# Toytiny/CMFlow

Measured on AMD Instinct MI355X. Metric: frame-pairs/sec CMFlow fwd+bwd, higher is better.
Workload: dtype f32; 1 GPU; cmflow fwd+bwd training (7 cross-modal losses + Adam, train-mode BN) step, N=256, B=64 per GPU (global 64), ball-query r=2/4/8/16 K=4/8/16/32, kNN K=8; synthetic clouds, seeded random-init weights; parallelism=dp1

## Files before the change

cmflow_amd/_lib.py:

```python
import ctypes
import os
import subprocess

import torch

_HERE = os.path.dirname(os.path.abspath(__file__))
SO_PATH = os.environ.get("CMF_LIB") or os.path.join(_HERE, "libcmflow_hip.so")

_vp, _ci, _cf, _ll = ctypes.c_void_p, ctypes.c_int, ctypes.c_float, ctypes.c_longlong

SIGNATURES = {
    "cmf_ball_query": [_ci, _ci, _ci, _cf, _ci, _vp, _vp, _vp, _vp],
    "cmf_ball_query_multi": [_ci, _ci, _ci, _ci, _vp, _vp, _ci, _vp, _vp, _vp, _ci, _vp],
    "cmf_setconv_queries": [_ci, _vp, _vp],
    "cmf_ball_query_multi_counted": [_ci, _ci, _ci, _ci, _vp, _vp, _ci, _vp, _vp, _vp, _vp, _vp, _vp],
    "cmf_setconv_queries_counted": [_ci, _vp, _vp, _vp],
    "cmf_knn_counted": [_ci, _ci, _ci, _ci, _vp, _vp, _vp, _vp, _vp, _vp],
    "cmf_global_max_cat_counted": [_ci, _ci, _ci, _vp, _ll, _vp, _ll, _vp, _vp, _vp],
    "cmf_ego_refine_counted": [_ci, _ci, _cf, _cf, _vp, _vp, _vp, _vp, _vp, _vp, _vp, _vp, _vp, _vp, _vp, _vp],
    "cmf_eval_metrics_counted": [_ci, _ci, _vp, _vp, _vp, _vp, _vp, _vp, _vp, _vp, _cf, _cf, _cf, _vp, _vp, _vp],
    "cmf_ego_refine_grad_counted": [_ci, _ci, _cf, _vp, _vp, _vp, _vp, _vp, _vp, _vp, _vp, _vp, _vp, _vp, _vp, _vp],
    "cmf_global_max_cat_grad_counted": [_ci, _ci, _ci, _vp, _ll, _vp, _vp, _ll, _vp, _vp],
    "cmf_radar_loss_counted_workspace": [_ci, _ci, _ci, _ci],
    "cmf_radar_loss_counted_workspace_tiled": [_ci, _ci, _ci, _ci],
# ... 51 lines not shown
    "cmf_three_interpolate_grad": [_ci, _ci, _ci, _ci, _vp, _vp, _vp, _vp, _vp],
    "cmf_bn_finalize": [_ci, _ci, ctypes.c_double, _vp, _vp, _vp, _cf, _cf, _vp, _vp, _vp, _vp, _vp, _vp, _vp, _vp],
    "cmf_colsum_finalize": [_ci, _ci, _vp, _vp, _vp, _vp, _vp],
    "cmf_group_affine": [_ci, _ci, _ci, _ci, _ci, _vp, _ci, _vp, _ci, _vp, _vp, _vp, _ci, _vp, _ci, _vp, _vp, _vp, _vp, _vp],
    "cmf_adam_step": [_ci, _vp, _vp, _ll, _vp, _vp, _vp, ctypes.c_double, ctypes.c_double, ctypes.c_double, ctypes.c_double, ctypes.c_double, _ll, _vp],
    "cmf_grad_norm_parts": [_ll],
    "cmf_grad_sumsq": [_ll, _vp, _vp, _vp],
    "cmf_grad_norm": [_ll, _vp, _vp, _vp, _vp],
    "cmf_adam_step_guarded": [_ci, _vp, _vp, _ll, _vp, _vp, _vp, ctypes.c_double, ctypes.c_double, ctypes.c_double, ctypes.c_double, ctypes.c_double, _ll,
                              ctypes.c_double, _ci, _vp, _vp, _vp],
    "cmf_adam_step_ema": [_ci, _vp, _vp, _ll, _vp, _vp, _vp, ctypes.c_double, ctypes.c_double, ctypes.c_double, ctypes.c_double, ctypes.c_double, _ll,
                          _vp, ctypes.c_double, _vp],
    "cmf_adam_step_guarded_ema": [_ci, _vp, _vp, _ll, _vp, _vp, _vp, ctypes.c_double, ctypes.c_double, ctypes.c_double, ctypes.c_double, ctypes.c_double,
                                  _ll, ctypes.c_double, _ci, _vp, _vp, _vp, ctypes.c_double, _vp],
    "cmf_param_exchange": [_ci, _vp, _vp, _ll, _vp, _vp],
    "cmf_group_prep": [_ci, _ci, _ci, _ci, _ci, _vp, _vp, _vp, _ci, _vp, _vp, _vp, _vp, _vp],
    "cmf_gemm_gather_affine": [_ci, _ci, _ci, _vp, _ll, _vp, _vp, _vp, _vp, _vp, _vp, _ll, _vp, _ll, _vp, _vp],
    "cmf_gemm_dx_gather": [_ci, _ci, _ci, _vp, _ll, _vp, _ll, _vp, _ll, _vp, _ll, _vp, _vp, _vp, _vp, _vp, _vp, _vp, _vp, _vp],
    "cmf_group_perm": [_ci, _ci, _vp, _vp, _vp, _vp, _vp, _vp, _vp],
    "cmf_gemm_dx_gather_sum": [_ci, _ci, _ci, _vp, _ll, _vp, _ll, _vp, _ll, _vp, _vp, _vp, _vp, _vp, _vp, _vp, _vp, _vp, _vp, _vp],
    "cmf_group_rows_grad_bn_cf_pieces": [_ci, _ci, _ci, _ci, _ci, _vp, _vp, _ll, _vp, _ll, _vp, _vp, _vp, _vp, _vp, _vp, _cf, _vp, _vp, _vp,
                                         _ci, _vp],
    "cmf_gemm_dw_gather_split": [_ci, _ci, _ll],
    "cmf_gemm_dw_gather_bn_bwd": [_ci, _ci, _ll, _vp, _ll, _vp, _ll, _vp, _vp, _vp, _vp, _vp, _ll, _vp, _ll, _vp, _vp, _vp, _vp, _vp, _vp, _ll,
                                  _ci, _vp, _ci, _vp],
    "cmf_gemm_dw_gather": [_ci, _ci, _ll, _vp, _ll, _vp, _ll, _vp, _vp, _vp, _vp, _vp, _vp, _ll, _ci, _vp, _ci, _vp],
    "cmf_colsum": [_ci, _ci, _vp, _vp, _ci, _vp, _vp, _vp],
    "cmf_setconv_dwx": [_ci, _cf, _ci, _vp, _vp, _vp, _vp, _vp, _vp, _ci, _ci, _vp],
    "cmf_group_rows_grad_bn": [_ci, _ci, _ci, _ci, _vp, _vp, _vp, _vp, _vp, _vp, _cf, _vp, _vp, _vp, _ci, _vp],
    "cmf_group_rows_grad_bn_cf": [_ci, _ci, _ci, _ci, _ci, _vp, _vp, _ll, _vp, _ll, _vp, _vp, _vp, _vp, _vp, _vp, _cf, _vp, _vp, _vp,
                                  _ci, _vp],
    "cmf_bn_relu_maxpool": [_ll, _ci, _ci, _vp, _vp, _vp, _vp, _ll, _vp, _vp],
    "cmf_maxpool_bwd": [_ll, _ci, _ci, _vp, _ll, _vp, _vp, _vp, _vp, _vp, _vp, _vp, _vp, _vp],
    "cmf_affine_relu": [_ll, _ci, _vp, _ll, _vp, _vp, _vp, _ll, _vp],
    "cmf_act_bwd_stats": [_ll, _ci, _vp, _ll, _vp, _ll, _vp, _vp, _vp, _vp, _vp, _vp, _vp],
    "cmf_bn_bwd_apply": [_ll, _ci, _vp, _vp, _ll, _vp, _vp, _vp, _vp, _vp],
    "cmf_maxpool_bwd_point": [_ll, _ci, _ci, _vp, _ll, _vp, _vp, _vp, _vp, _vp, _vp, _vp, _vp, _vp],
    "cmf_thin_bwd_layer_pooled": [_ll, _ci, _ci, _ci, _vp, _vp, _vp, _vp, _vp, _vp, _vp, _vp, _vp, _vp, _vp, _vp, _vp, _vp, _vp, _vp,
                                  _ci, _vp, _vp],
    "cmf_thin_bwd_wide_supported": [_ci, _ci],
    "cmf_thin_bwd_wide_slabs": [_ll, _ci, _vp],
    "cmf_thin_bwd_wide_layer": [_ll, _ci, _vp, _ll, _vp, _vp, _ci, _vp, _ll, _vp, _vp, _vp, _vp, _vp, _ll, _vp, _ll,
                                _vp, _vp, _vp, _vp, _vp, _ll, _vp, _vp, _ll, _ci, _vp, _vp],
    "cmf_thin_bwd_supported": [_ci, _ci],
    "cmf_thin_bwd_slabs": [_ll, _vp],
    "cmf_thin_bwd_layer": [_ll, _ci, _ci, _vp, _ll, _vp, _ll, _vp, _vp, _vp, _vp, _vp, _ll, _vp, _ll, _ci,
                           _vp, _vp, _vp, _vp, _vp, _vp, _ll, _vp, _vp, _ll, _ci, _vp, _vp],
    "cmf_weighted_ksum": [_ll, _ci, _ci, _ci, _ci, _vp, _vp, _vp, _vp, _vp],
    "cmf_weighted_ksum_grad_tiles": [_ci],
    "cmf_weighted_ksum_grad": [_ll, _ci, _ci, _ci, _ci, _ci, _vp, _vp, _vp, _vp, _vp, _vp, _vp, _vp],
    "cmf_weightnet_ksum_tiles": [_ci],
    "cmf_weightnet_ksum": [_ll, _ci, _ci, _ci, _ci, _vp, _vp, _vp, _vp, _vp, _vp, _vp],
    "cmf_weightnet_ksum_grad": [_ll, _ci, _ci, _ci, _ci, _ci, _vp, _ll, _vp, _vp, _vp, _vp, _vp, _vp, _vp, _vp, _vp],
    "cmf_global_max_cat": [_ci, _ci, _ci, _vp, _ll, _vp, _ll, _vp, _vp],
    "cmf_stack_first_conv": [_ci, _ci, _ci, _ci, _ci, _vp, _vp, _vp],
    "cmf_unstack_first_conv_grad": [_ci, _ci, _ci, _ci, _ci, _vp, _vp, _vp],
    "cmf_global_max_cat_grad": [_ci, _ci, _ci, _vp, _ll, _vp, _vp, _ll, _vp],
    "cmf_mem_stats": [],
    "cmf_radar_loss_workspace_nb": [_ci, _ci, _ci],
    "cmf_radar_loss_workspace_tiled": [_ci, _ci, _ci],
    "cmf_radar_loss": [_vp, _vp],
    "cmf_radar_loss_tiled": [_vp, _vp],
    "cmf_pseudo_labels": [_ci, _ci, _vp, _vp, _vp, _vp, _vp, _vp, _cf, _vp, _vp, _vp, _vp],
    "cmf_draw_batch": [_ci, _ci, _ci, _ci, _vp, _vp, _vp, _vp, _vp, _vp, _vp, ctypes.c_ulonglong, ctypes.c_ulonglong,
                       _vp, _vp, _vp, _vp, _vp, _vp, _vp, _vp, _vp, _vp, _vp, _vp, _vp, _vp],
    "cmf_draw_batch_at": [_ci, _ci, _ci, _ci, _ci, _vp, _vp, _vp, _vp, _vp, _vp, _vp, ctypes.c_ulonglong, ctypes.c_ulonglong,
                          _vp, _vp, _vp, _vp, _vp, _vp, _vp, _vp, _vp, _vp, _vp, _vp, _vp, _vp],
    "cmf_draw_frames": [_ci, _ci, _ci, _ci, _vp, _vp, _vp, _vp, _vp, _vp, _vp,
                        _vp, _vp, _vp, _vp, _vp, _vp, _vp, _vp, _vp, _vp, _vp, _vp, _vp, _vp],
    "cmf_augment_batch": [_ci, _ci, _ci, _ci, ctypes.c_ulonglong, ctypes.c_ulonglong, ctypes.c_double, _ci, _vp, _vp, _vp, _vp, _vp, _vp, _vp, _vp],
    "cmf_prepare_count": [_ci, _ci, _vp, _vp, _vp, _vp, _ci, _ci, _ci, ctypes.c_double, ctypes.c_double, _vp, _vp, _vp, _vp],
    "cmf_prepare_scans": [_ci, _ci, _ci, _vp, _vp, _vp, _vp, _ci, _ci, _ci, ctypes.c_double, ctypes.c_double, _vp, _vp, _vp, _vp],
    "cmf_prepare_pairs": [_ci, _ci, _vp, _vp, _vp, _vp, _vp, _vp, _vp, _vp, _vp, _vp, _ci, _vp, _ci, _ci, _vp, _vp, _vp],
    "cmf_pack_results": [_ci, _ci, _ci, _vp, _vp, _vp, _ll, _vp, _vp, _vp, _vp, _vp, _vp, _vp, _vp, _vp, _vp, _vp, _vp],
    "cmf_eval_metrics_frames": [_ci, _ci, _vp, _vp, _vp, _vp, _vp, _vp, _vp, _vp, _cf, _cf, _cf, _ci, _vp, _vp, _vp, _vp],
    "cmf_pose_chain": [_ci, _ci, _vp, _vp, _vp, _vp],
    "cmf_debug_spin": [_cf, _vp],
    "cmf_eval_metrics": [_ci, _ci, _vp, _vp, _vp, _vp, _vp, _vp, _vp, _cf, _cf, _cf, _vp, _vp, _vp],
}
RESTYPES = {"cmf_mem_stats": _ll, "cmf_radar_loss_counted_workspace": _ll, "cmf_radar_loss_counted_workspace_tiled": _ll,
            "cmf_radar_loss_workspace_nb": _ll, "cmf_radar_loss_workspace_tiled": _ll, "cmf_gemm_trace_read": _ll, "cmf_gemm_profile_records": _ll}


class GemmLaunchRecord(ctypes.Structure):
    _fields_ = [("M", _ci), ("N", _ci), ("K", _ci), ("layout", _ci), ("split_k", _ci), ("kind", _ci), ("bm", _ci), ("bn", _ci),
                ("ms", _cf)]


class SetConvDesc(ctypes.Structure):
    _fields_ = [("B", _ci), ("N", _ci), ("S", _ci), ("O1", _ci), ("C", _ci * 5), ("radius", _cf), ("training", _ci),
                ("eps", _cf * 6), ("momentum", _cf * 6),
                ("xyz", _vp), ("y", _vp), ("ldy", _ll), ("wx", _vp), ("ldwx", _ll), ("w", _vp * 5),
                ("gamma", _vp * 6), ("beta", _vp * 6), ("rmean", _vp * 6), ("rvar", _vp * 6), ("nbt", _vp * 6),
                ("saved", _vp), ("scratch", _vp), ("out", _vp), ("ldo", _ll),
                ("dout", _vp), ("lddout", _ll), ("dy", _vp), ("lddy", _ll), ("dwx", _vp), ("lddwx", _ll), ("acc_wx", _ci),
                ("dw", _vp * 5), ("acc_w", _ci * 5), ("dgamma", _vp * 6), ("dbeta", _vp * 6), ("acc_bn", _ci * 6),
                ("inference", _ci), ("idx_ready", _ci)]


class MlpDesc(ctypes.Structure):
    _fields_ = [("M", _ll), ("L", _ci), ("C", _ci * 5), ("training", _ci), ("eps", _cf * 4), ("momentum", _cf * 4),
                ("x", _vp), ("ldx", _ll), ("w", _vp * 4), ("gamma", _vp * 4), ("beta", _vp * 4),
                ("rmean", _vp * 4), ("rvar", _vp * 4), ("nbt", _vp * 4), ("saved", _vp), ("scratch", _vp),
                ("out", _vp), ("ldo", _ll), ("dout", _vp), ("lddout", _ll), ("dx", _vp), ("lddx", _ll),
                ("dw", _vp * 4), ("acc_w", _ci * 4), ("dgamma", _vp * 4), ("dbeta", _vp * 4), ("acc_bn", _ci * 4)]

# ... 131 lines not shown
```

cmflow_amd/csrc/wsum.hip:

```cpp
#include "cmf_common.h"
#include "../../include/cmflow_hip.h"

constexpr int WS_THREADS = 256;

template <int KU>
__global__ __launch_bounds__(WS_THREADS) void wsum_fwd_kernel(
    long long M, int K, int C, int n1, int n_src, const float *__restrict__ w, const float *__restrict__ x,
    const int *__restrict__ idx, float *__restrict__ out)
{
    const int cv = C / 4;
    const long long total = M * cv;
    for (long long t = (long long)blockIdx.x * WS_THREADS + threadIdx.x; t < total; t += (long long)gridDim.x * WS_THREADS) {
        const long long m = t / cv;
        const int c = (int)(t - m * cv) * 4;
        const float *wp = w + (m * K) * C + c;
        const long long src_base = idx ? (m / n1) * n_src : 0;
        float4 acc = make_float4(0.f, 0.f, 0.f, 0.f);
        for (int k0 = 0; k0 < K; k0 += KU) {
            float4 wv[KU], xv[KU];
#pragma unroll
            for (int u = 0; u < KU; ++u) {
                const int k = k0 + u;
                if (k < K) {
                    wv[u] = *(const float4 *)(wp + (long long)k * C);
// ... 232 lines not shown
            q2[i] = keep + __shfl_xor(send, 16, 64);
        }
        {
            const float keep = up3 ? q2[1] : q2[0], send = up3 ? q2[0] : q2[1];
            q1 = keep + __shfl_xor(send, 8, 64);
        }
        q1 += __shfl_xor(q1, 4, 64);
        q1 += __shfl_xor(q1, 2, 64);
        q1 += __shfl_xor(q1, 1, 64);
        if ((lane & 7) == 0) sred[it & 1][wave][(lane >> 5) * 4 + ((lane >> 4) & 1) * 2 + ((lane >> 3) & 1)] = q1;
        __syncthreads();
        if (tid < R * WN_J) {
            const int rr = tid / WN_J, j = tid % WN_J;
            if (row0 + rr < MK) {
                float s = sred[it & 1][rr * wpr][j];
                for (int w = 1; w < wpr; ++w) s += sred[it & 1][rr * wpr + w][j];
                if (leaky & 4) {
                    s = h[(long long)(row0 + rr) * WN_J + j] > 0.f ? s : 0.f;
                    dbh += s;
                }
                dh[(long long)(row0 + rr) * WN_J + j] = s;
            }
        }
    }
    float *prow = part + (long long)blockIdx.x * (C * (WN_J + 2) + WN_J);
    {
        __syncthreads();
        float *fl = (float *)fold;
        if (tid < R * WN_J) fl[tid] = dbh;
        __syncthreads();
        if (tid < WN_J) {
            float t = fl[tid];
            for (int rr = 1; rr < R; ++rr) t += fl[rr * WN_J + tid];
            prow[C * (WN_J + 2) + tid] = t;
        }
    }
#pragma unroll
    for (int q = 0; q < 10; ++q) {
        float4 v;
        if (q < 8) { const int i = q >> 1, j = (q & 1) * 4; v = make_float4(dW[i][j], dW[i][j + 1], dW[i][j + 2], dW[i][j + 3]); }
        else if (q == 8) v = make_float4(db[0], db[1], db[2], db[3]);
        else v = make_float4(cs[0], cs[1], cs[2], cs[3]);
        __syncthreads();
        fold[tid] = v;
        __syncthreads();
        if (r == 0) {
            for (int rr = 1; rr < R; ++rr) { const float4 o = fold[tid + rr * cv]; v.x += o.x; v.y += o.y; v.z += o.z; v.w += o.w; }
            if (q < 8) *(float4 *)(prow + (c + (q >> 1)) * WN_J + (q & 1) * 4) = v;
            else *(float4 *)(prow + C * WN_J + (q - 8) * C + c) = v;
        }
    }
}

extern "C" int cmf_weightnet_ksum_tiles(int C)
{
    return (C == 256 || C == 512 || C == 1024) ? WN_TILES : 0;
}

extern "C" int cmf_weightnet_ksum(long long M, int K, int C, int n1, int n_src, const float *h, const float *Wl, const float *bl,
                                  const float *x, const int *idx, float *out, void *stream)
{
    CMF_CHECK_ARG(M >= 0 && K > 0 && cmf_weightnet_ksum_tiles(C) > 0 && M * K < (1LL << 31));
    if (M == 0) return 0;
    CMF_CHECK_ARG(h && Wl && bl && x && out && (!idx || (n1 > 0 && n_src > 0)));
    CMF_CHECK_ARG((((uintptr_t)h | (uintptr_t)Wl | (uintptr_t)x | (uintptr_t)out) & 15) == 0);
    const int R = WS_THREADS / (C / 4);
    const long long want = (M + R - 1) / R;
    const int grid = (int)(want < 2048 ? want : 2048);
    hipLaunchKernelGGL(wn_ksum_fwd_kernel, dim3(grid), dim3(WS_THREADS), 0, (hipStream_t)stream, (int)M, K, C, n1, n_src, h, Wl, bl, x, idx, out);
    return cmf_launch_status();
}

extern "C" int cmf_weightnet_ksum_grad(long long M, int K, int C, int n1, int n_src, int leaky, const float *dcost, long long ldd, const float *h,
                                       const float *Wl, const float *bl, const float *x, const int *idx, float *dx, float *dh,
                                       float *part, void *stream)
{
    CMF_CHECK_ARG(M >= 0 && K > 0 && cmf_weightnet_ksum_tiles(C) > 0 && M * K < (1LL << 31));
    CMF_CHECK_ARG(dcost && h && Wl && bl && x && dx && dh && part && (!idx || (n1 > 0 && n_src > 0)) && ldd >= C && ldd % 4 == 0);
    CMF_CHECK_ARG((((uintptr_t)h | (uintptr_t)Wl | (uintptr_t)x | (uintptr_t)dcost | (uintptr_t)dx | (uintptr_t)dh | (uintptr_t)part) & 15) == 0);
    hipLaunchKernelGGL(wn_ksum_bwd_kernel, dim3(WN_TILES), dim3(WS_THREADS), 0, (hipStream_t)stream, (int)M, K, C, n1, n_src, leaky, dcost, ldd, h,
                       Wl, bl, x, idx, dx, dh, part);
    return cmf_launch_status();
}
```

cmflow_amd/fused_blocks.py:

```python
import ctypes
import os

import torch
from torch.autograd import Function

from . import _lib
from . import pointnet2_utils as pointutils
from .fused import Neighbors, gemm, group_rows

_f32, _i32 = torch.float32, torch.int32
L = _lib.lib


def _p(t):
    return None if t is None else t.data_ptr()


def _tiles(M):
    return (M + 127) // 128


class BNState:
    __slots__ = ("a", "c", "mean", "invstd", "training", "count")

# ... 1128 lines not shown
        n_src = nbr.n if nbr is not None else 0
        part, db = None, None
        want_db = ctx.x_bias is not None and len(ctx.needs_input_grad) > 5 and ctx.needs_input_grad[5] and need_x
        tiles = L().cmf_weighted_ksum_grad_tiles(C) if want_db else 0
        if tiles > 0:
            part = torch.empty(tiles, 1, C, dtype=_f32, device=weights.device)
        _lib.check(L().cmf_weighted_ksum_grad(B * N1, K, C, N1, n_src, int(leaky), _p(dcost), _p(weights), _p(x), idx,
                                              _p(dw), _p(dx), _p(part), _lib.stream_ptr()), "cmf_weighted_ksum_grad")
        if want_db:
            if part is not None:
                sink = grad_sink(ctx.x_bias)
                sums = colsum_n(part, C, sink, None)
                db = None if sink is not None else sums.view(-1)
            else:
                db = dx.view(-1, C).sum(0)
        if nbr is not None and need_x:
            off, inv = nbr.inverse()
            dp = torch.empty(B, nbr.n, C, dtype=_f32, device=weights.device)
            _lib.check(L().cmf_group_rows_grad(B, nbr.n, C, C, N1 * K, 0, _p(dx), _p(off), _p(inv), _p(dp), _lib.stream_ptr()),
                       "cmf_group_rows_grad")
            dx = dp
        return dw, dx, None, None, None, db


class WeightNetKSumFn(Function):

    @staticmethod
    def supported(C, J):
        return J == 8 and L().cmf_weightnet_ksum_tiles(int(C)) > 0

    @staticmethod
    def forward(ctx, h, wl, bl, x, nbr, leaky, x_bias=None, h_bias=None):
        B, N1, K, J = h.shape
        C = wl.shape[0]
        h, wl, bl, x = h.contiguous(), wl.contiguous(), bl.contiguous(), x.contiguous()
        out = torch.empty(B, N1, C, dtype=_f32, device=h.device)
        idx = _lib.dev_ptr(nbr.idx, torch.int32) if nbr is not None else None
        n_src = nbr.n if nbr is not None else 0
        _lib.check(L().cmf_weightnet_ksum(B * N1, K, C, N1, n_src, _p(h), _p(wl), _p(bl), _p(x), idx, _p(out), _lib.stream_ptr()),
                   "cmf_weightnet_ksum")
        ctx.saved = (h, wl, bl, x, nbr, int(bool(leaky)) | (4 if h_bias is not None else 0))
        ctx.params = (wl, bl, x_bias, h_bias)
        return out

    @staticmethod
    def backward(ctx, dcost):
        h, wl, bl, x, nbr, leaky = ctx.saved
        B, N1, K, J = h.shape
        C = wl.shape[0]
        dev = h.device
        if not (dcost.stride(2) == 1 and dcost.stride(0) == N1 * dcost.stride(1) and dcost.stride(1) % 4 == 0
                and dcost.data_ptr() % 16 == 0):
            dcost = dcost.contiguous()
        dx = torch.empty(B, N1, K, C, dtype=_f32, device=dev)
        dh = torch.empty_like(h)
        part = torch.empty(L().cmf_weightnet_ksum_tiles(C), C * (J + 2) + J, dtype=_f32, device=dev)
        idx = _lib.dev_ptr(nbr.idx, torch.int32) if nbr is not None else None
        n_src = nbr.n if nbr is not None else 0
        _lib.check(L().cmf_weightnet_ksum_grad(B * N1, K, C, N1, n_src, leaky, dcost.data_ptr(), dcost.stride(1), _p(h), _p(wl), _p(bl), _p(x), idx,
                                               _p(dx), _p(dh), _p(part), _lib.stream_ptr()), "cmf_weightnet_ksum_grad")
        sums = colsum_n(part)
        grads = [sums[:C * J].view(C, J), sums[C * J:C * J + C], sums[C * J + C:C * J + 2 * C] if ctx.params[2] is not None else None,
                 sums[C * (J + 2):] if ctx.params[3] is not None else None]
        sinks = [grad_sink(p) if p is not None else None for p in ctx.params]
        pairs = [(s.view(-1), g.reshape(-1)) for s, g in zip(sinks, grads) if s is not None and g is not None]
        if pairs:
            torch._foreach_add_([s for s, _ in pairs], [g for _, g in pairs])
        dwl, dbl, dxb, dhb = [None if (s is not None or g is None) else g for s, g in zip(sinks, grads)]
        if nbr is not None:
            off, inv = nbr.inverse()
            dp = torch.empty(B, nbr.n, C, dtype=_f32, device=dev)
            _lib.check(L().cmf_group_rows_grad(B, nbr.n, C, C, N1 * K, 0, _p(dx), _p(off), _p(inv), _p(dp), _lib.stream_ptr()),
                       "cmf_group_rows_grad")
            dx = dp
        return dh, dwl, dbl, dx, None, None, dxb, dhb


class GlobalMaxCatFn(Function):

    @staticmethod
    def forward(ctx, f):
        B, N, C = f.shape
        f = f.contiguous()
        out = torch.empty(B, N, 2 * C, dtype=_f32, device=f.device)
        arg = torch.empty(B, C, dtype=torch.int32, device=f.device)
        _lib.check(L().cmf_global_max_cat(B, N, C, _p(f), C, _p(out), 2 * C, _p(arg), _lib.stream_ptr()), "cmf_global_max_cat")
        ctx.arg = arg
        return out

    @staticmethod
    def backward(ctx, dout):
        B, C = ctx.arg.shape
        N = dout.shape[1]
        if not (dout.stride(2) == 1 and dout.stride(0) == N * dout.stride(1) and dout.stride(1) % 4 == 0 and dout.data_ptr() % 16 == 0):
            dout = dout.contiguous()
        df = torch.empty(B, N, C, dtype=_f32, device=dout.device)
        _lib.check(L().cmf_global_max_cat_grad(B, N, C, dout.data_ptr(), dout.stride(1), _p(ctx.arg), _p(df), C, _lib.stream_ptr()),
                   "cmf_global_max_cat_grad")
        return df


def global_max_cat(f):
    return GlobalMaxCatFn.apply(f)


class GlobalMaxCatCountedFn(Function):

    @staticmethod
    def forward(ctx, f, counts):
        B, N, C = f.shape
        f = f.contiguous()
        out = torch.empty(B, N, 2 * C, dtype=_f32, device=f.device)
        arg = torch.empty(B, C, dtype=torch.int32, device=f.device)
        _lib.check(L().cmf_global_max_cat_counted(B, N, C, _p(f), C, _p(out), 2 * C, _p(arg), _lib.dev_ptr(counts, torch.int32),
                                                  _lib.stream_ptr()), "cmf_global_max_cat_counted")
        ctx.arg, ctx.counts = arg, counts
        return out

    @staticmethod
    def backward(ctx, dout):
        B, C = ctx.arg.shape
        N = dout.shape[1]
# ... 20 lines not shown
```

include/cmflow_hip.h:

```cpp
#ifndef CMFLOW_HIP_H
#define CMFLOW_HIP_H

#ifdef __cplusplus
extern "C" {
#endif


int cmf_ball_query(int b, int n, int m, float radius, int nsample,
                   const float *new_xyz, const float *xyz, int *idx, void *stream);
int cmf_ball_query_multi(int b, int n, int m, int nq, const float *radii, const int *nsamples, int nclouds,
                         const float *const *new_xyz, const float *const *xyz, int *const *idx, int zero_empty, void *stream);

int cmf_group_points(int b, int c, int n, int npoints, int nsample,
                     const float *points, const int *idx, float *out, void *stream);

int cmf_group_points_grad(int b, int c, int n, int npoints, int nsample,
                          const float *grad_out, const int *idx, float *grad_points, void *stream);

int cmf_query_and_group(int b, int n, int m, float radius, int nsample, int c, int use_xyz,
                        const float *new_xyz, const float *xyz, const float *features, int *idx, float *out, void *stream);


int cmf_knn(int b, int n, int s, int nsample, const float *xyz, const float *new_xyz,
            int *idx, float *dist, void *stream);
// ... 207 lines not shown
                      void *stream);
int cmf_adam_step_guarded_ema(int n_tensors, const long long *offsets, float *const *params, long long total, const float *grad, float *m,
                              float *v, double lr, double beta1, double beta2, double eps, double weight_decay, long long step,
                              double max_grad_norm, int skip_nonfinite, const double *partials, double *record, float *ema,
                              double ema_decay, void *stream);
int cmf_param_exchange(int n_tensors, const long long *offsets, float *const *params, long long total, float *flat, void *stream);

int cmf_setconv_bn_offsets(const cmf_setconv_desc *d, long long *offsets6);

typedef struct cmf_mlp_desc {
    long long M; int L; int C[5]; int training;
    float eps[4], momentum[4];
    const float *x; long long ldx;
    const float *w[4];
    const float *gamma[4], *beta[4];
    float *rmean[4], *rvar[4]; long long *nbt[4];
    float *saved, *scratch;
    float *out; long long ldo;
    const float *dout; long long lddout;
    float *dx; long long lddx;
    float *dw[4]; int acc_w[4];
    float *dgamma[4], *dbeta[4]; int acc_bn[4];
} cmf_mlp_desc;
int cmf_mlp_sizes(const cmf_mlp_desc *d, long long *saved_floats, long long *scratch_fwd, long long *scratch_bwd);
int cmf_mlp_forward(const cmf_mlp_desc *d, void *stream);
int cmf_mlp_backward(const cmf_mlp_desc *d, void *stream);

typedef struct cmf_bn_update_entry {
    float *rmean, *rvar; long long *nbt;
    int C; float momentum, eps; double count;
    long long offset;
} cmf_bn_update_entry;
int cmf_bn_running_update(int n_entries, const cmf_bn_update_entry *table, int n_calls, const float *saved0,
                          const float *saved1, void *stream);

int cmf_setconv_forward_heads_multi(int n, const cmf_setconv_desc *descs, void *const *streams);
int cmf_setconv_forward_bodies_batched(int n, const cmf_setconv_desc *descs);
int cmf_setconv_backward_bodies_batched(int n, const cmf_setconv_desc *descs);
int cmf_setconv_tail_forward(int n, const cmf_setconv_desc *descs, void *stream);
int cmf_setconv_tail_backward(int n, const cmf_setconv_desc *descs, void *stream);
int cmf_setconv_backward_bodies_multi(int n, const cmf_setconv_desc *descs, void *const *streams);

int cmf_weighted_ksum(long long M, int K, int C, int n1, int n_src, const float *w, const float *x, const int *idx,
                      float *out, void *stream);
int cmf_weighted_ksum_grad_tiles(int C);
int cmf_weighted_ksum_grad(long long M, int K, int C, int n1, int n_src, int leaky, const float *dcost, const float *w,
                           const float *x, const int *idx, float *dw, float *dx, float *dx_colsum, void *stream);
int cmf_weightnet_ksum_tiles(int C);
int cmf_weightnet_ksum(long long M, int K, int C, int n1, int n_src, const float *h, const float *Wl, const float *bl,
                       const float *x, const int *idx, float *out, void *stream);
int cmf_weightnet_ksum_grad(long long M, int K, int C, int n1, int n_src, int leaky, const float *dcost, long long ldd, const float *h,
                            const float *Wl, const float *bl, const float *x, const int *idx, float *dx, float *dh,
                            float *part, void *stream);

int cmf_global_max_cat(int B, int N, int C, const float *f, long long ldf, float *out, long long ldo, int *arg, void *stream);
int cmf_global_max_cat_grad(int B, int N, int C, const float *dout, long long ldd, const int *arg, float *df, long long ldf,
                            void *stream);

int cmf_stack_first_conv(int n_w, int O1, int cin, int n_tail, int Kp, const float *const *w, float *wf, void *stream);
int cmf_unstack_first_conv_grad(int n_w, int O1, int cin, int n_tail, int Kp, const float *dwf, float *const *g, void *stream);

#define CMF_RADAR_LOSS_MAX_N 65536
typedef struct cmf_radar_loss_desc {
    int B, N;
    const float *pc1, *pc2, *pred_f, *gt_f;
    const float *vel1, *mseg_pre, *mseg_gt, *dyn_mask, *radar_u, *radar_v;
    const float *opt;
    const float *pre_trans, *gt_trans;
    const float *camera_inverse;
    const float *t_camera_radar;
    float w_self, w_em, w_ms, w_opt, w_dyn;
    float zeta, alpha; int num_nb; float lower_bound;
    int self_only;
    float *items;
    float *d_pred_f, *d_pre_trans, *d_mseg_pre;
    float *workspace;
    const float *t_camera_radar_batch;
} cmf_radar_loss_desc;
long long cmf_radar_loss_workspace_nb(int b, int n, int num_nb);
int cmf_radar_loss(const cmf_radar_loss_desc *d, void *stream);
int cmf_radar_loss_tiled(const cmf_radar_loss_desc *d, void *stream);
long long cmf_radar_loss_workspace_tiled(int b, int n, int num_nb);

int cmf_eval_metrics(int b, int n, const float *pc, const float *pred, const float *labels, const float *mask,
                     const float *pred_m, const float *gt_trans, const float *pred_trans,
                     float r_res, float theta_res, float phi_res, double *metrics, double *workspace, void *stream);

int cmf_pseudo_labels(int b, int n, const float *pc1, const float *gt_trans, const float *vel1, const float *interval,
                      const float *fg_mask, const float *flow_label, float vr_thres,
                      float *dyn_mask, float *mseg_gt, float *residual, void *stream);

int cmf_debug_spin(float microseconds, void *stream);

int cmf_ball_query_multi_counted(int b, int n, int m, int nq, const float *radii, const int *nsamples, int nclouds,
                                 const float *const *new_xyz, const float *const *xyz, int *const *idx,
                                 const int *const *n_ctr, const int *const *n_src, void *stream);
int cmf_setconv_queries_counted(int n, const cmf_setconv_desc *descs, const int *const *counts, void *stream);
int cmf_knn_counted(int b, int n, int s, int nsample, const float *xyz, const float *new_xyz, const int *n_src,
                    int *idx, float *dist, void *stream);
int cmf_global_max_cat_counted(int B, int N, int C, const float *f, long long ldf, float *out, long long ldo, int *arg,
                               const int *cnt, void *stream);
int cmf_ego_refine_counted(int b, int n, float eps, float thres, const float *pc1, const float *flow, const float *score,
                           const int *cnt, float *W, float *Bm, float *trans, double *aux, float *sf, unsigned char *mask,
                           float *stat, void *stream);
int cmf_eval_metrics_counted(int b, int n, const int *cnt, const float *pc, const float *pred, const float *labels, const float *mask,
                             const float *pred_m, const float *gt_trans, const float *pred_trans,
// ... 90 lines not shown
```

Before: 3444 frame-pairs/s.

## Fuse weightnet ksum backward with neighbor scatter via inverse index lists

Adds a wave-per-row weightnet ksum backward kernel for C=256/512 with register-resident weights and a depth-2 load prefetch. Adds a scatter variant that walks each source point's inverse neighbor list and accumulates dx straight into per-point gradients. This removes the B×N1×K×C intermediate dx tensor and the separate group_rows_grad pass. In exchange the code is more complex, depends on the inverse-list layout, and risks load imbalance across waves when neighbor lists vary in length.

Result: no change. 3464 frame-pairs/s, median of 6 (+0.6%).

```diff
diff --git a/cmflow_amd/_lib.py b/cmflow_amd/_lib.py
--- a/cmflow_amd/_lib.py
+++ b/cmflow_amd/_lib.py
@@ -127,6 +127,8 @@
     "cmf_weightnet_ksum_tiles": [_ci],
     "cmf_weightnet_ksum": [_ll, _ci, _ci, _ci, _ci, _vp, _vp, _vp, _vp, _vp, _vp, _vp],
     "cmf_weightnet_ksum_grad": [_ll, _ci, _ci, _ci, _ci, _ci, _vp, _ll, _vp, _vp, _vp, _vp, _vp, _vp, _vp, _vp, _vp],
+    "cmf_weightnet_ksum_scatter_tiles": [_ci],
+    "cmf_weightnet_ksum_grad_scatter": [_ll, _ci, _ci, _ci, _ci, _ci, _vp, _ll, _vp, _vp, _vp, _vp, _vp, _vp, _vp, _vp, _vp, _vp],
     "cmf_global_max_cat": [_ci, _ci, _ci, _vp, _ll, _vp, _ll, _vp, _vp],
     "cmf_stack_first_conv": [_ci, _ci, _ci, _ci, _ci, _vp, _vp, _vp],
     "cmf_unstack_first_conv_grad": [_ci, _ci, _ci, _ci, _ci, _vp, _vp, _vp],
diff --git a/cmflow_amd/csrc/wsum.hip b/cmflow_amd/csrc/wsum.hip
--- a/cmflow_amd/csrc/wsum.hip
+++ b/cmflow_amd/csrc/wsum.hip
@@ -308,9 +308,12 @@
     }
 }
 
+int cmf_wn_ksum_bwd_wave(int M, int K, int C, int n1, int n_src, int leaky, const float *dcost, long long ldd, const float *h, const float *Wl,
+                         const float *bl, const float *x, const int *idx, float *dx, float *dh, float *part, hipStream_t st);
+
 extern "C" int cmf_weightnet_ksum_tiles(int C)
 {
-    return (C == 256 || C == 512 || C == 1024) ? WN_TILES : 0;
+    return cmf_weightnet_ksum_scatter_tiles(C) > 0 ? cmf_weightnet_ksum_scatter_tiles(C) : C == 1024 ? WN_TILES : 0;
 }
 
 extern "C" int cmf_weightnet_ksum(long long M, int K, int C, int n1, int n_src, const float *h, const float *Wl, const float *bl,
@@ -334,6 +337,7 @@
     CMF_CHECK_ARG(M >= 0 && K > 0 && cmf_weightnet_ksum_tiles(C) > 0 && M * K < (1LL << 31));
     CMF_CHECK_ARG(dcost && h && Wl && bl && x && dx && dh && part && (!idx || (n1 > 0 && n_src > 0)) && ldd >= C && ldd % 4 == 0);
     CMF_CHECK_ARG((((uintptr_t)h | (uintptr_t)Wl | (uintptr_t)x | (uintptr_t)dcost | (uintptr_t)dx | (uintptr_t)dh | (uintptr_t)part) & 15) == 0);
+    if (C != 1024) return cmf_wn_ksum_bwd_wave((int)M, K, C, n1, n_src, leaky, dcost, ldd, h, Wl, bl, x, idx, dx, dh, part, (hipStream_t)stream);
     hipLaunchKernelGGL(wn_ksum_bwd_kernel, dim3(WN_TILES), dim3(WS_THREADS), 0, (hipStream_t)stream, (int)M, K, C, n1, n_src, leaky, dcost, ldd, h,
                        Wl, bl, x, idx, dx, dh, part);
     return cmf_launch_status();
diff --git a/cmflow_amd/csrc/wsum_wave.hip b/cmflow_amd/csrc/wsum_wave.hip
--- /dev/null
+++ b/cmflow_amd/csrc/wsum_wave.hip
@@ -0,0 +1,311 @@
+#include "cmf_common.h"
+#include "../../include/cmflow_hip.h"
+
+constexpr int WS_THREADS = 256;
+constexpr int WN_J = 8;
+
+constexpr int WNW_TILES = 512;
+constexpr int WNW_DEPTH = 2;
+constexpr int WNS_DEPTH = 2;
+
+template <int CPL>
+__device__ __forceinline__ int wnw_channel(int lane, int i) { return (i >> 2) * 256 + lane * 4 + (i & 3); }
+
+template <int CPL>
+__device__ __forceinline__ void wnw_slot(const float (&W)[CPL][WN_J], const float (&b)[CPL], const float (&hv)[WN_J], const float4 (&g4)[CPL / 4],
+                                         const float4 (&x4)[CPL / 4], int leaky, float (&dW)[CPL][WN_J], float (&db)[CPL], float (&cs)[CPL],
+                                         float (&d)[CPL], float (&p)[WN_J])
+{
+#pragma unroll
+    for (int j = 0; j < WN_J; ++j) p[j] = 0.f;
+#pragma unroll
+    for (int i = 0; i < CPL; ++i) {
+        const float4 gv = g4[i >> 2], xw = x4[i >> 2];
+        const float g = (i & 3) == 0 ? gv.x : (i & 3) == 1 ? gv.y : (i & 3) == 2 ? gv.z : gv.w;
+        const float xv = (i & 3) == 0 ? xw.x : (i & 3) == 1 ? xw.y : (i & 3) == 2 ? xw.z : xw.w;
+        float pre = b[i];
+#pragma unroll
+        for (int j = 0; j < WN_J; ++j) pre = fmaf(hv[j], W[i][j], pre);
+        const float e = pre > 0.f ? g * xv : 0.f;
+        float dd = __fmul_rn(g, fmaxf(pre, 0.f));
+        if (leaky & 1) dd = xv > 0.f ? dd : __fmul_rn(0.1f, dd);
+        d[i] = dd;
+        cs[i] += dd;
+        db[i] += e;
+#pragma unroll
+        for (int j = 0; j < WN_J; ++j) {
+            dW[i][j] = fmaf(e, hv[j], dW[i][j]);
+            p[j] = fmaf(e, W[i][j], p[j]);
+        }
+    }
+}
+
+__device__ __forceinline__ void wnw_dh(const float (&p)[WN_J], float h_lane, int lane, int leaky, float *__restrict__ dh_row, float &dbh)
+{
+    float q4[4], q2[2], q1;
+    const bool up5 = lane & 32, up4 = lane & 16, up3 = lane & 8;
+#pragma unroll
+    for (int i = 0; i < 4; ++i) {
+        const float keep = up5 ? p[i + 4] : p[i], send = up5 ? p[i] : p[i + 4];
+        q4[i] = keep + __shfl_xor(send, 32, 64);
+    }
+#pragma unroll
+    for (int i = 0; i < 2; ++i) {
+        const float keep = up4 ? q4[i + 2] : q4[i], send = up4 ? q4[i] : q4[i + 2];
+        q2[i] = keep + __shfl_xor(send, 16, 64);
+    }
+    {
+        const float keep = up3 ? q2[1] : q2[0], send = up3 ? q2[0] : q2[1];
+        q1 = keep + __shfl_xor(send, 8, 64);
+    }
+    q1 += __shfl_xor(q1, 4, 64);
+    q1 += __shfl_xor(q1, 2, 64);
+    q1 += __shfl_xor(q1, 1, 64);
+    if (leaky & 4) {
+        q1 = h_lane > 0.f ? q1 : 0.f;
+        if ((lane & 7) == 0) dbh += q1;
+    }
+    if ((lane & 7) == 0) dh_row[lane >> 3] = q1;
+}
+
+__device__ __forceinline__ void wnw_h_row(float h_lane, float (&hv)[WN_J])
+{
+#pragma unroll
+    for (int j = 0; j < WN_J; ++j) hv[j] = __builtin_bit_cast(float, __builtin_amdgcn_readlane(__builtin_bit_cast(int, h_lane), 8 * j));
+}
+
+template <int CPL>
+__device__ __forceinline__ void wnw_fold(const float (&dW)[CPL][WN_J], const float (&db)[CPL], const float (&cs)[CPL], float dbh, int lane, int wave,
+                                         float *__restrict__ prow)
+{
+    constexpr int C = CPL * 64;
+    __shared__ float4 fold[2][WS_THREADS];
+    __shared__ float fl[WS_THREADS / 64][WN_J];
+    const int tid = wave * 64 + lane;
+    if ((lane & 7) == 0) fl[wave][lane >> 3] = dbh;
+    __syncthreads();
+    if (tid < WN_J) prow[C * (WN_J + 2) + tid] = ((fl[0][tid] + fl[1][tid]) + fl[2][tid]) + fl[3][tid];
+#pragma unroll
+    for (int q = 0; q < 2 * CPL + CPL / 2; ++q) {
+        float4 v;
+        float *dst;
+        if (q < 2 * CPL) {
+            const int i = q >> 1, j = (q & 1) * 4;
+            v = make_float4(dW[i][j], dW[i][j + 1], dW[i][j + 2], dW[i][j + 3]);
+            dst = prow + wnw_channel<CPL>(lane, i) * WN_J + j;
+        } else {
+            const int r = q - 2 * CPL, which = r / (CPL / 4), i = (r % (CPL / 4)) * 4;
+            v = which == 0 ? make_float4(db[i], db[i + 1], db[i + 2], db[i + 3]) : make_float4(cs[i], cs[i + 1], cs[i + 2], cs[i + 3]);
+            dst = prow + C * WN_J + which * C + wnw_channel<CPL>(lane, i);
+        }
+        fold[q & 1][tid] = v;
+        __syncthreads();
+        if (wave == 0) {
+#pragma unroll
+            for (int w = 1; w < WS_THREADS / 64; ++w) { const float4 o = fold[q & 1][lane + w * 64]; v.x += o.x; v.y += o.y; v.z += o.z; v.w += o.w; }
+            *(float4 *)dst = v;
+        }
+    }
+}
+
+template <int CPL>
+__device__ __forceinline__ void wnw_load_w(const float *__restrict__ Wl, const float *__restrict__ bl, int lane, float (&W)[CPL][WN_J], float (&b)[CPL])
+{
+#pragma unroll
+    for (int i = 0; i < CPL; ++i) {
+        const int ch = wnw_channel<CPL>(lane, i);
+        const float4 lo = *(const float4 *)(Wl + (long long)ch * WN_J), hi = *(const float4 *)(Wl + (long long)ch * WN_J + 4);
+        W[i][0] = lo.x; W[i][1] = lo.y; W[i][2] = lo.z; W[i][3] = lo.w; W[i][4] = hi.x; W[i][5] = hi.y; W[i][6] = hi.z; W[i][7] = hi.w;
+        b[i] = bl[ch];
+    }
+}
+
+template <int CPL>
+__global__ __launch_bounds__(WS_THREADS, 2) void wn_ksum_bwd_wave_kernel(
+    int M, int K, int n1, int n_src, int leaky, const float *__restrict__ dcost, long long ldd, const float *__restrict__ h,
+    const float *__restrict__ Wl, const float *__restrict__ bl, const float *__restrict__ x, const int *__restrict__ idx,
+    float *__restrict__ dx, float *__restrict__ dh, float *__restrict__ part)
+{
+    constexpr int C = CPL * 64, V = CPL / 4, D = WNW_DEPTH;
+    const int lane = threadIdx.x & 63, wave = __builtin_amdgcn_readfirstlane((int)threadIdx.x >> 6);
+    const unsigned lo = lane * 4;
+    const long long gw = (long long)blockIdx.x * (WS_THREADS / 64) + wave, nw = (long long)gridDim.x * (WS_THREADS / 64);
+    const long long MK = (long long)M * K;
+    const int s0 = (int)(MK * gw / nw), s1 = (int)(MK * (gw + 1) / nw);
+    float W[CPL][WN_J], b[CPL], dW[CPL][WN_J], db[CPL], cs[CPL], dbh = 0.f;
+    wnw_load_w<CPL>(Wl, bl, lane, W, b);
+#pragma unroll
+    for (int i = 0; i < CPL; ++i) {
+        db[i] = 0.f; cs[i] = 0.f;
+#pragma unroll
+        for (int j = 0; j < WN_J; ++j) dW[i][j] = 0.f;
+    }
+    float4 gq[D][V], xq[D][V];
+    float hq[D];
+    auto request = [&](int mk, float4 (&g4)[V], float4 (&x4)[V], float &h_lane) {
+        const int m = mk / K;
+        const long long row = idx ? (long long)(m / n1) * n_src + idx[mk] : mk;
+        const float *gr = dcost + (long long)m * ldd, *xp = x + row * C;
+#pragma unroll
+        for (int v = 0; v < V; ++v) {
+            g4[v] = *(const float4 *)(gr + (lo + v * 256));
+            x4[v] = *(const float4 *)(xp + (lo + v * 256));
+        }
+        h_lane = (h + (long long)mk * WN_J)[lane >> 3];
+    };
+#pragma unroll
+    for (int u = 0; u < D; ++u)
+        if (s0 + u < s1) request(s0 + u, gq[u], xq[u], hq[u]);
+    for (int s = s0; s < s1; s += D) {
+#pragma unroll
+        for (int u = 0; u < D; ++u) {
+            const int mk = s + u;
+            if (mk < s1) {
+                float d[CPL], p[WN_J], hv[WN_J];
+                wnw_h_row(hq[u], hv);
+                wnw_slot<CPL>(W, b, hv, gq[u], xq[u], leaky, dW, db, cs, d, p);
+                float *dr = dx + (long long)mk * C;
+#pragma unroll
+                for (int v = 0; v < V; ++v) *(float4 *)(dr + (lo + v * 256)) = make_float4(d[4 * v], d[4 * v + 1], d[4 * v + 2], d[4 * v + 3]);
+                wnw_dh(p, hq[u], lane, leaky, dh + (long long)mk * WN_J, dbh);
+                if (mk + D < s1) request(mk + D, gq[u], xq[u], hq[u]);
+            }
+        }
+    }
+    wnw_fold<CPL>(dW, db, cs, dbh, lane, wave, part + (long long)blockIdx.x * (C * (WN_J + 2) + WN_J));
+}
+
+template <int CPL>
+__global__ __launch_bounds__(WS_THREADS, 2) void wn_ksum_bwd_scatter_kernel(
+    int B, int n1, int K, int n_src, int leaky, const float *__restrict__ dcost, long long ldd, const float *__restrict__ h,
+    const float *__restrict__ Wl, const float *__restrict__ bl, const float *__restrict__ x, const int *__restrict__ offsets,
+    const int *__restrict__ inv, float *__restrict__ dp, float *__restrict__ dh, float *__restrict__ part)
+{
+    constexpr int C = CPL * 64, V = CPL / 4, D = WNS_DEPTH;
+    const int lane = threadIdx.x & 63, wave = __builtin_amdgcn_readfirstlane((int)threadIdx.x >> 6);
+    const unsigned lo = lane * 4;
+    const long long gw = (long long)blockIdx.x * (WS_THREADS / 64) + wave, nw = (long long)gridDim.x * (WS_THREADS / 64);
+    const long long P = (long long)B * n_src;
+    const int entries = n1 * K;
+    const int p0 = (int)(P * gw / nw), p1 = (int)(P * (gw + 1) / nw);
+    float W[CPL][WN_J], b[CPL], dW[CPL][WN_J], db[CPL], cs[CPL], dbh = 0.f;
+    wnw_load_w<CPL>(Wl, bl, lane, W, b);
+#pragma unroll
+    for (int i = 0; i < CPL; ++i) {
+        db[i] = 0.f; cs[i] = 0.f;
+#pragma unroll
+        for (int j = 0; j < WN_J; ++j) dW[i][j] = 0.f;
+    }
+    if (p0 < p1) {
+        auto list_end = [&](int p) {
+            const int bs = p / n_src, j = p - bs * n_src;
+            return bs * entries + offsets[(long long)bs * (n_src + 1) + j + 1];
+        };
+        auto list_begin = [&](int p) {
+            const int bs = p / n_src, j = p - bs * n_src;
+            return bs * entries + offsets[(long long)bs * (n_src + 1) + j];
+        };
+        const int t0 = __builtin_amdgcn_readfirstlane(list_begin(p0)), t1 = __builtin_amdgcn_readfirstlane(list_end(p1 - 1));
+        int pc = p0, endv = list_end(min(pc + lane, p1 - 1));
+        int tc = t0, ev = 0, evn = 0;
+        if (t0 < t1) { ev = inv[min(tc + lane, t1 - 1)]; evn = inv[min(tc + 64 + lane, t1 - 1)]; }
+        float4 gq[D][V], xr[V], xn[V];
+        float hq[D], acc[CPL];
+        auto request = [&](int t, float4 (&g4)[V], float &h_lane) {
+            const int e = t - tc < 64 ? __builtin_amdgcn_readlane(ev, t - tc) : __builtin_amdgcn_readlane(evn, t - tc - 64);
+            const int mk = (t / entries) * entries + e, m = mk / K;
+            const float *gr = dcost + (long long)m * ldd;
+#pragma unroll
+            for (int v = 0; v < V; ++v) g4[v] = *(const float4 *)(gr + (lo + v * 256));
+            h_lane = (h + (long long)mk * WN_J)[lane >> 3];
+        };
+        auto load_x = [&](int p, float4 (&x4)[V]) {
+            const float *xp = x + (long long)p * C;
+#pragma unroll
+            for (int v = 0; v < V; ++v) x4[v] = *(const float4 *)(xp + (lo + v * 256));
+        };
+        auto store_dp = [&](int p) {
+            float *dr = dp + (long long)p * C;
+#pragma unroll
+            for (int v = 0; v < V; ++v) *(float4 *)(dr + (lo + v * 256)) = make_float4(acc[4 * v], acc[4 * v + 1], acc[4 * v + 2], acc[4 * v + 3]);
+#pragma unroll
+            for (int i = 0; i < CPL; ++i) acc[i] = 0.f;
+        };
+#pragma unroll
+        for (int i = 0; i < CPL; ++i) acc[i] = 0.f;
+        int p = p0, end = __builtin_amdgcn_readlane(endv, 0);
+        load_x(p0, xr);
+        load_x(min(p0 + 1, p1 - 1), xn);
+#pragma unroll
+        for (int u = 0; u < D; ++u)
+            if (t0 + u < t1) request(t0 + u, gq[u], hq[u]);
+        for (int ts = t0; ts < t1; ts += D) {
+#pragma unroll
+            for (int u = 0; u < D; ++u) {
+                const int t = ts + u;
+                if (t < t1) {
+                    while (t == end) {
+                        store_dp(p);
+                        ++p;
+#pragma unroll
+                        for (int v = 0; v < V; ++v) xr[v] = xn[v];
+                        if (p + 1 < p1) load_x(p + 1, xn);
+                        if (p - pc == 64) { pc = p; endv = list_end(min(pc + lane, p1 - 1)); }
+                        end = __builtin_amdgcn_readlane(endv, p - pc);
+                    }
+                    const int e = __builtin_amdgcn_readlane(ev, t - tc);
+                    const int mk = (t / entries) * entries + e;
+                    float d[CPL], pj[WN_J], hv[WN_J];
+                    wnw_h_row(hq[u], hv);
+                    wnw_slot<CPL>(W, b, hv, gq[u], xr, leaky, dW, db, cs, d, pj);
+#pragma unroll
+                    for (int i = 0; i < CPL; ++i) acc[i] = __fadd_rn(acc[i], d[i]);
+                    wnw_dh(pj, hq[u], lane, leaky, dh + (long long)mk * WN_J, dbh);
+                    if (t + 1 - tc == 64) { tc += 64; ev = evn; evn = inv[min(tc + 64 + lane, t1 - 1)]; }
+                    if (t + D < t1) request(t + D, gq[u], hq[u]);
+                }
+            }
+        }
+        for (;;) {
+            store_dp(p);
+            if (++p >= p1) break;
+        }
+    }
+    wnw_fold<CPL>(dW, db, cs, dbh, lane, wave, part + (long long)blockIdx.x * (C * (WN_J + 2) + WN_J));
+}
+
+int cmf_wn_ksum_bwd_wave(int M, int K, int C, int n1, int n_src, int leaky, const float *dcost, long long ldd, const float *h, const float *Wl,
+                         const float *bl, const float *x, const int *idx, float *dx, float *dh, float *part, hipStream_t st)
+{
+    CMF_CHECK_ARG(C == 256 || C == 512);
+    if (C == 512)
+        hipLaunchKernelGGL(wn_ksum_bwd_wave_kernel<8>, dim3(WNW_TILES), dim3(WS_THREADS), 0, st, M, K, n1, n_src, leaky, dcost, ldd, h, Wl, bl, x, idx,
+                           dx, dh, part);
+    else
+        hipLaunchKernelGGL(wn_ksum_bwd_wave_kernel<4>, dim3(WNW_TILES), dim3(WS_THREADS), 0, st, M, K, n1, n_src, leaky, dcost, ldd, h, Wl, bl, x, idx,
+                           dx, dh, part);
+    return cmf_launch_status();
+}
+
+extern "C" int cmf_weightnet_ksum_scatter_tiles(int C)
+{
+    return (C == 256 || C == 512) ? WNW_TILES : 0;
+}
+
+extern "C" int cmf_weightnet_ksum_grad_scatter(long long M, int K, int C, int n1, int n_src, int leaky, const float *dcost, long long ldd,
+                                               const float *h, const float *Wl, const float *bl, const float *x, const int *offsets, const int *inv,
+                                               float *dp, float *dh, float *part, void *stream)
+{
+    CMF_CHECK_ARG(M >= 0 && K > 0 && cmf_weightnet_ksum_scatter_tiles(C) > 0 && M * K < (1LL << 31) && n1 > 0 && n_src > 0 && M % n1 == 0);
+    CMF_CHECK_ARG((M / n1) * n_src < (1LL << 31) && (long long)n1 * K < (1LL << 31));
+    CMF_CHECK_ARG(dcost && h && Wl && bl && x && offsets && inv && dp && dh && part && ldd >= C && ldd % 4 == 0);
+    CMF_CHECK_ARG((((uintptr_t)h | (uintptr_t)Wl | (uintptr_t)x | (uintptr_t)dcost | (uintptr_t)dp | (uintptr_t)dh | (uintptr_t)part) & 15) == 0);
+    const int B = (int)(M / n1);
+    if (C == 512)
+        hipLaunchKernelGGL(wn_ksum_bwd_scatter_kernel<8>, dim3(WNW_TILES), dim3(WS_THREADS), 0, (hipStream_t)stream, B, n1, K, n_src, leaky, dcost,
+                           ldd, h, Wl, bl, x, offsets, inv, dp, dh, part);
+    else
+        hipLaunchKernelGGL(wn_ksum_bwd_scatter_kernel<4>, dim3(WNW_TILES), dim3(WS_THREADS), 0, (hipStream_t)stream, B, n1, K, n_src, leaky, dcost,
+                           ldd, h, Wl, bl, x, offsets, inv, dp, dh, part);
+    return cmf_launch_status();
+}
diff --git a/cmflow_amd/fused_blocks.py b/cmflow_amd/fused_blocks.py
--- a/cmflow_amd/fused_blocks.py
+++ b/cmflow_amd/fused_blocks.py
@@ -1204,13 +1204,22 @@
         if not (dcost.stride(2) == 1 and dcost.stride(0) == N1 * dcost.stride(1) and dcost.stride(1) % 4 == 0
                 and dcost.data_ptr() % 16 == 0):
             dcost = dcost.contiguous()
-        dx = torch.empty(B, N1, K, C, dtype=_f32, device=dev)
         dh = torch.empty_like(h)
-        part = torch.empty(L().cmf_weightnet_ksum_tiles(C), C * (J + 2) + J, dtype=_f32, device=dev)
-        idx = _lib.dev_ptr(nbr.idx, torch.int32) if nbr is not None else None
-        n_src = nbr.n if nbr is not None else 0
-        _lib.check(L().cmf_weightnet_ksum_grad(B * N1, K, C, N1, n_src, leaky, dcost.data_ptr(), dcost.stride(1), _p(h), _p(wl), _p(bl), _p(x), idx,
-                                               _p(dx), _p(dh), _p(part), _lib.stream_ptr()), "cmf_weightnet_ksum_grad")
+        scatter = nbr is not None and L().cmf_weightnet_ksum_scatter_tiles(C) > 0
+        if scatter:
+            off, inv = nbr.inverse()
+            part = torch.empty(L().cmf_weightnet_ksum_scatter_tiles(C), C * (J + 2) + J, dtype=_f32, device=dev)
+            dx = torch.empty(B, nbr.n, C, dtype=_f32, device=dev)
+            _lib.check(L().cmf_weightnet_ksum_grad_scatter(B * N1, K, C, N1, nbr.n, leaky, dcost.data_ptr(), dcost.stride(1), _p(h), _p(wl), _p(bl),
+                                                           _p(x), _p(off), _p(inv), _p(dx), _p(dh), _p(part), _lib.stream_ptr()),
+                       "cmf_weightnet_ksum_grad_scatter")
+        else:
+            dx = torch.empty(B, N1, K, C, dtype=_f32, device=dev)
+            part = torch.empty(L().cmf_weightnet_ksum_tiles(C), C * (J + 2) + J, dtype=_f32, device=dev)
+            idx = _lib.dev_ptr(nbr.idx, torch.int32) if nbr is not None else None
+            n_src = nbr.n if nbr is not None else 0
+            _lib.check(L().cmf_weightnet_ksum_grad(B * N1, K, C, N1, n_src, leaky, dcost.data_ptr(), dcost.stride(1), _p(h), _p(wl), _p(bl), _p(x),
+                                                   idx, _p(dx), _p(dh), _p(part), _lib.stream_ptr()), "cmf_weightnet_ksum_grad")
         sums = colsum_n(part)
         grads = [sums[:C * J].view(C, J), sums[C * J:C * J + C], sums[C * J + C:C * J + 2 * C] if ctx.params[2] is not None else None,
                  sums[C * (J + 2):] if ctx.params[3] is not None else None]
@@ -1219,7 +1228,7 @@
         if pairs:
             torch._foreach_add_([s for s, _ in pairs], [g for _, g in pairs])
         dwl, dbl, dxb, dhb = [None if (s is not None or g is None) else g for s, g in zip(sinks, grads)]
-        if nbr is not None:
+        if nbr is not None and not scatter:
             off, inv = nbr.inverse()
             dp = torch.empty(B, nbr.n, C, dtype=_f32, device=dev)
             _lib.check(L().cmf_group_rows_grad(B, nbr.n, C, C, N1 * K, 0, _p(dx), _p(off), _p(inv), _p(dp), _lib.stream_ptr()),
diff --git a/include/cmflow_hip.h b/include/cmflow_hip.h
--- a/include/cmflow_hip.h
+++ b/include/cmflow_hip.h
@@ -283,6 +283,10 @@
 int cmf_weightnet_ksum_grad(long long M, int K, int C, int n1, int n_src, int leaky, const float *dcost, long long ldd, const float *h,
                             const float *Wl, const float *bl, const float *x, const int *idx, float *dx, float *dh,
                             float *part, void *stream);
+int cmf_weightnet_ksum_scatter_tiles(int C);
+int cmf_weightnet_ksum_grad_scatter(long long M, int K, int C, int n1, int n_src, int leaky, const float *dcost, long long ldd,
+                                    const float *h, const float *Wl, const float *bl, const float *x, const int *offsets, const int *inv,
+                                    float *dp, float *dh, float *part, void *stream);
 
 int cmf_global_max_cat(int B, int N, int C, const float *f, long long ldf, float *out, long long ldo, int *arg, void *stream);
 int cmf_global_max_cat_grad(int B, int N, int C, const float *dout, long long ldd, const int *arg, float *df, long long ldf,
```
